# hotchpotch/open_provence

Hardware: AMD Instinct MI355X
Metric: query-context pairs/sec @ seq_len 512, xsmall-v1 (higher is better)
Workload: dtype fp16 single pass (11 significant bits per operand), fp32 accumulate

## Files before the change

### open_provence_amd/csrc/op_api.hip

```cpp
#include "../../include/open_provence_hip.h"

#include <hip/hip_runtime.h>

#include <algorithm>
#include <cmath>
#include <cstdarg>
#include <cstdio>
#include <cstdlib>
#include <cstring>
#include <string>
#include <vector>

#define OPK_PACK_KERNELS 1
#include "op_internal.h"
#include "op_sets.h"
#include "opk_small.hip.h"
#include "opk_padded.hip.h"
#include "opk_tiled.hip.h"

using namespace opk;
using opl::Policy;
using namespace ops;

namespace {
// ... 312 lines not shown
  ChunkPass(op_handle* h_, Launcher& L_, const Workspace& ws_, const int32_t* ids_dev_, const int32_t* cu_dev_, int s0_, int ns_, int rows_,
            int max_len_, int total_tokens_, const AttnPlan& plan_, float* prune_out_, float* rank_out_, float* keep_prob_,
            const HiddenReq* hid_)
      : h(h_), L(L_), ws(ws_), ids_dev(ids_dev_), cu_dev(cu_dev_), s0(s0_), ns(ns_), rows(rows_), max_len(max_len_),
        total_tokens(total_tokens_), plan(plan_), prune_out(prune_out_), rank_out(rank_out_), keep_prob(keep_prob_), hid(hid_) {
    H = h->H;
    I = h->I;
    fp_layout = h->row_path || h->panel_path;
    r_pad = fp_layout ? align_up(rows, ROW_BM) : align_up(rows + 64, 256);
    m_tiles = r_pad / GEMM_BM;
    row_blocks = (unsigned)((r_pad + 3) / 4);
    st = L.stream;
    const KernelSet& ks = *h->ks;
    E = h->eff;
    pi = ks.pi;
    V = opl::kPolicies[pi];
    o_f8 = ks.side == FMT_F8;
    f16 = ks.side == FMT_F16;
    attn16 = o_f8 && ks.attn == FMT_F16;
    auto extra = [](int v, int e, int bit) { return (v & bit) != 0 && (e & bit) == 0; };
    clr_q = !attn16 && extra(V.qk, E.qk, 1);
    clr_k = !attn16 && extra(V.qk, E.qk, 2);
    clr_v = !attn16 && extra(V.pv, E.pv, 2);
    clr_o = extra(V.attn_out, E.attn_out, 1);
    clr_h = extra(V.mlp_out, E.mlp_out, 1);
    clr_ln_attn = extra(V.wqkv, E.wqkv, 1);
    clr_ln_mlp = extra(V.wi, E.wi, 1);
    zero_p_lo = !attn16 && extra(V.pv, E.pv, 1);
    split = (E.wqkv | E.qk | E.pv | E.attn_out | E.wi | E.mlp_out) != 0;
    wi8 = !o_f8 && ks.wi == FMT_F8 && ks.mlp != FMT_F8;
    wlo8 = ks.wlo;
    for (int li = 0; li < h->N; ++li) mlp8[li] = mlp_by_layer(ks) && (li >= 64 || ((h->mlp_layers >> li) & 1ull) != 0);
    range_flagged = h->panel_path && (o_f8 || ks.mlp == FMT_F8);
    fmt_base = f16 ? PF_PK16 : PF_PK;
    fmt_f8 = h->row_path ? PF_ROW_F8A : PF_PANEL16;
    fmt_side = o_f8 ? fmt_f8 : fmt_base;
    fmt_wi = (o_f8 || wi8) ? fmt_f8 : fmt_base;
    embed_in_qkv0 = h->row_path && !h->capture && !(h->cfg.flags & OP_FLAG_NO_HEAD_FUSION);
    plane_bytes = (size_t)r_pad * H * sizeof(u16);
    q_tiles = (max_len + ATT_BQ - 1) / ATT_BQ;
    small_blocks = (r_pad / ROW_BM) <= h->n_cus && !(h->cfg.flags & OP_FLAG_NO_SMALL_BLOCKS);
    row_grid = (unsigned)(r_pad / (small_blocks ? 64 : ROW_BM));
    layer_fused = h->row_path && h->set >= 0 && opl::has_row_layer_fused(pi) && !(h->cfg.flags & OP_FLAG_NO_LAYER_FUSION);
    head_in_last_layer = layer_fused && h->cfg.pooling != OP_POOL_MEAN && !h->capture && !(h->cfg.flags & OP_FLAG_NO_HEAD_FUSION);
    pair_layers = layer_fused && H == 256 && I % 64 == 0 && !split && !h->capture &&
                  !(h->cfg.flags & (OP_FLAG_NO_LAYER_PAIRS | OP_FLAG_LAYER_8X16 | OP_FLAG_LAYER_M32)) &&
                  weight(0, W_ATTN_OUT, f16 ? PF_PAIR16 : PF_PAIR) != nullptr;
  }

  u16* weight(int li, Weight w, PackFmt f) const { return h->layers[li].pack[w][f]; }

  int prologue() {
    OP_TRY(L.begin(PK_ROWMAP));
    hipLaunchKernelGGL(seq_offsets_kernel, dim3(1), dim3(1024), 0, st, cu_dev, s0, ns, ROW_ALIGN, ROW_ALIGN, ws.roff);
    if (fp_layout) {
      hipLaunchKernelGGL(seq_offsets_kernel, dim3(1), dim3(1024), 0, st, cu_dev, s0, ns, plan.waves_g * 32, 1, ws.qboff);
      hipLaunchKernelGGL(seq_offsets_kernel, dim3(1), dim3(1024), 0, st, cu_dev, s0, ns, 128, 1, ws.qboff_l);
    }
    hipLaunchKernelGGL(row_map_kernel, dim3((unsigned)((r_pad + 255) / 256)), dim3(256), 0, st, cu_dev, s0, ns, ws.roff,
                       r_pad, ws.row_seq, ws.row_pos, ws.row_tok);
    OP_TRY(L.end());

    if (range_flagged) OP_HIP(h, hipMemsetAsync(ws.range_flag, 0, sizeof(int), st));
    if (fp_layout && o_f8) {
      const size_t n16 = (size_t)((r_pad - rows) / 16);
      if (n16) OP_HIP(h, hipMemsetAsync(ws.o_hi + (size_t)(rows / 16) * (H / 32) * 512, 0, n16 * (H / 32) * 512 * sizeof(u16), st));
      if (n16) OP_HIP(h, hipMemsetAsync(ws.o_lo + (size_t)(rows / 16) * h->nh * 512, 0, n16 * h->nh * 512 * sizeof(u16), st));
    } else if (fp_layout) {
      const size_t tail_off = (size_t)(rows / 16) * (H / 32) * 2 * 512;
      const size_t tail_bytes = (size_t)((r_pad - rows) / 16) * (H / 32) * 2 * 512 * sizeof(u16);
      if (tail_bytes) OP_HIP(h, hipMemsetAsync(ws.o_hi + tail_off, 0, tail_bytes, st));
    } else {
      const size_t tail_off = (size_t)rows * H;
      const size_t tail_bytes = (size_t)(r_pad - rows) * H * sizeof(u16);
      if (tail_bytes) OP_HIP(h, hipMemsetAsync(ws.o_hi + tail_off, 0, tail_bytes, st));
      if (tail_bytes && split) OP_HIP(h, hipMemsetAsync(ws.o_lo + tail_off, 0, tail_bytes, st));
    }

    if (!embed_in_qkv0) {
      OP_TRY(L.begin(PK_EMBED_LN));
      if (split)
        hipLaunchKernelGGL((embed_ln_kernel<true>), dim3(row_blocks), dim3(256), 0, st, ids_dev, ws.row_tok, h->emb,
                           h->emb_norm, h->cfg.norm_eps, H, r_pad, h->V, ws.x, ws.ln_hi, ws.ln_lo);
      else
        hipLaunchKernelGGL((embed_ln_kernel<false>), dim3(row_blocks), dim3(256), 0, st, ids_dev, ws.row_tok, h->emb,
                           h->emb_norm, h->cfg.norm_eps, H, r_pad, h->V, ws.x, ws.ln_hi, ws.ln_lo);
      OP_TRY(L.end());
    }
    return OP_OK;
  }

  int capture(int index) {
    if (!h->capture) return OP_OK;
    OP_TRY(L.begin(PK_CAPTURE));
    hipLaunchKernelGGL(capture_rows_kernel, dim3(row_blocks), dim3(256), 0, st, ws.x, ws.row_tok, H, r_pad,
                       h->capture + (size_t)index * total_tokens * H);
    return L.end();
  }

  void* hidden_entry(int index) const {
    if (!hid || hid->slot[index] < 0) return nullptr;
    return hid->out + (size_t)hid->slot[index] * hid->entry_bytes;
  }
  int hidden(int index, const float* ln = nullptr) {
    void* dst = hidden_entry(index);
    if (!dst) return OP_OK;
    OP_TRY(L.begin(PK_CAPTURE));
    hipLaunchKernelGGL(hidden_rows_kernel, dim3(row_blocks), dim3(256), 0, st, ws.x, ln, h->cfg.norm_eps, H, r_pad,
                       ws.row_tok, ws.row_seq, ws.row_pos, s0, hid->pad, hid->bf16, dst);
    return L.end();
  }

  int attention(bool is_global) {
// ... 1614 lines not shown
```

### open_provence_amd/csrc/opk_small.hip.h

```cpp
#pragma once

#include "opk_common.hip.h"

namespace opk {

__global__ __launch_bounds__(1024) void seq_offsets_kernel(const int32_t* __restrict__ cu, int s0, int ns, int unit,
                                                           int scale, int32_t* __restrict__ roff) {
  __shared__ int sh[1024];
  __shared__ int carry;
  const int tid = threadIdx.x;
  if (tid == 0) carry = 0;
  __syncthreads();
  for (int base = 0; base < ns; base += 1024) {
    const int i = base + tid;
    int v = 0;
    if (i < ns) {
      const int len = cu[s0 + i + 1] - cu[s0 + i];
      v = (len + unit - 1) / unit * scale;
    }
    sh[tid] = v;
    __syncthreads();
    for (int off = 1; off < 1024; off <<= 1) {
      const int t = tid >= off ? sh[tid - off] : 0;
      __syncthreads();
      sh[tid] += t;
      __syncthreads();
    }
    const int incl = sh[tid];
    const int c = carry;
    if (i < ns) roff[i] = c + incl - v;
    __syncthreads();
    if (tid == 1023) carry = c + incl;
    __syncthreads();
  }
  if (tid == 0) roff[ns] = carry;
}

__global__ void row_map_kernel(const int32_t* __restrict__ cu, int s0, int ns, const int32_t* __restrict__ roff,
                               int r_pad, int32_t* __restrict__ row_seq, int32_t* __restrict__ row_pos,
                               int32_t* __restrict__ row_tok) {
  const int r = blockIdx.x * blockDim.x + threadIdx.x;
  if (r >= r_pad) return;
  const int total = roff[ns];
  if (r >= total) {
    row_seq[r] = -1;
    row_pos[r] = -1;
    row_tok[r] = -1;
    return;
  }
  int lo = 0, hi = ns - 1;
  while (lo < hi) {
    const int mid = (lo + hi + 1) >> 1;
    if (roff[mid] <= r) lo = mid; else hi = mid - 1;
  }
  const int pos = r - roff[lo];
  const int start = cu[s0 + lo];
  const int len = cu[s0 + lo + 1] - start;
  row_seq[r] = lo;
  if (pos < len) {
    row_pos[r] = pos;
    row_tok[r] = start + pos;
  } else {
    row_pos[r] = -1;
    row_tok[r] = -1;
  }
}

constexpr int LN_MAX_CHUNKS = 4;

struct RowVec {
  float4 v[LN_MAX_CHUNKS];
};

__device__ __forceinline__ void row_load(const float* __restrict__ src, int H, int lane, RowVec& rv) {
  const int nchunk = H >> 2;
#pragma unroll
  for (int k = 0; k < LN_MAX_CHUNKS; ++k) {
    const int c = lane + 64 * k;
    rv.v[k] = (c < nchunk) ? reinterpret_cast<const float4*>(src)[c] : make_float4(0.f, 0.f, 0.f, 0.f);
  }
}

__device__ __forceinline__ void row_layer_norm(RowVec& rv, const float* __restrict__ w, int H, int lane, float eps) {
  const int nchunk = H >> 2;
  float s = 0.f;
#pragma unroll
  for (int k = 0; k < LN_MAX_CHUNKS; ++k) s += (rv.v[k].x + rv.v[k].y) + (rv.v[k].z + rv.v[k].w);
  const float mean = wave_sum(s) / (float)H;
  float q = 0.f;
#pragma unroll
  for (int k = 0; k < LN_MAX_CHUNKS; ++k) {
    const int c = lane + 64 * k;
    if (c < nchunk) {
      const float a = rv.v[k].x - mean, b = rv.v[k].y - mean, cc = rv.v[k].z - mean, d = rv.v[k].w - mean;
      q += (a * a + b * b) + (cc * cc + d * d);
    }
  }
  const float var = wave_sum(q) / (float)H;
  const float rstd = 1.0f / sqrtf(var + eps);
#pragma unroll
  for (int k = 0; k < LN_MAX_CHUNKS; ++k) {
    const int c = lane + 64 * k;
    if (c < nchunk) {
      const float4 ww = reinterpret_cast<const float4*>(w)[c];
      rv.v[k].x = (rv.v[k].x - mean) * rstd * ww.x;
      rv.v[k].y = (rv.v[k].y - mean) * rstd * ww.y;
      rv.v[k].z = (rv.v[k].z - mean) * rstd * ww.z;
      rv.v[k].w = (rv.v[k].w - mean) * rstd * ww.w;
    }
  }
}
// ... 99 lines not shown
                                                             const int32_t* __restrict__ row_tok,
                                                             const int32_t* __restrict__ row_seq,
                                                             const int32_t* __restrict__ row_pos,
                                                             const float* __restrict__ pw, const float* __restrict__ pb,
                                                             float* __restrict__ prune_out, float* __restrict__ keep_prob,
                                                             int pre_norm, int keep_all_rows, float* __restrict__ cls,
                                                             float* __restrict__ capture, const int* __restrict__ range_flag) {
  const int lane = threadIdx.x & 63;
  const int row = blockIdx.x * 4 + (threadIdx.x >> 6);
  if (row >= r_pad) return;
  const int tok = row_tok[row];
  if (tok < 0) return;
  RowVec rv;
  row_load(x + (size_t)row * H, H, lane, rv);
  const int nchunk = H >> 2;
  float d0 = 0.f, d1 = 0.f;
  auto head_dot = [&]() {
#pragma unroll
    for (int k = 0; k < LN_MAX_CHUNKS; ++k) {
      const int c = lane + 64 * k;
      if (c < nchunk) {
        const float4 w0 = reinterpret_cast<const float4*>(pw)[c];
        const float4 w1 = reinterpret_cast<const float4*>(pw + H)[c];
        d0 += (rv.v[k].x * w0.x + rv.v[k].y * w0.y) + (rv.v[k].z * w0.z + rv.v[k].w * w0.w);
        d1 += (rv.v[k].x * w1.x + rv.v[k].y * w1.y) + (rv.v[k].z * w1.z + rv.v[k].w * w1.w);
      }
    }
  };
  if (pre_norm) head_dot();
  row_layer_norm(rv, lnw, H, lane, eps);
  if (!pre_norm) head_dot();
  d0 = wave_sum(d0);
  d1 = wave_sum(d1);
  if (lane == 0) {
    const float poison = (range_flag != nullptr && *range_flag != 0) ? __builtin_nanf("") : 0.f;
    const float l0 = d0 + pb[0] + poison, l1 = d1 + pb[1] + poison;
    prune_out[(size_t)tok * 2 + 0] = l0;
    prune_out[(size_t)tok * 2 + 1] = l1;
    if (keep_prob) keep_prob[tok] = 1.0f / (1.0f + expf(l0 - l1));
  }
  if (keep_all_rows) row_store_f32(rv, x + (size_t)row * H, H, lane);
  if (row_pos[row] == 0) row_store_f32(rv, cls + (size_t)row_seq[row] * H, H, lane);
  if (capture) row_store_f32(rv, capture + (size_t)tok * H, H, lane);
}

__device__ __forceinline__ float block_sum_256(float v, float* red) {
  v = wave_sum(v);
  const int wave = threadIdx.x >> 6, lane = threadIdx.x & 63;
  __syncthreads();
  if (lane == 0) red[wave] = v;
  __syncthreads();
  return (red[0] + red[1]) + (red[2] + red[3]);
}

__global__ __launch_bounds__(256) void rank_head_kernel(const float* __restrict__ cls, const float* __restrict__ y,
                                                        const int32_t* __restrict__ cu, int s0,
                                                        const int32_t* __restrict__ roff, int mean_pool, int H, int nl,
                                                        const float* __restrict__ dense_t,
                                                        const float* __restrict__ head_norm, float eps,
                                                        const float* __restrict__ cls_w, const float* __restrict__ cls_b,
                                                        float* __restrict__ rank_out, const int* __restrict__ range_flag) {
  const bool poisoned = range_flag != nullptr && *range_flag != 0;
  __shared__ float pooled[1024];
  __shared__ float z[1024];
  __shared__ float red[4];
  const int s = blockIdx.x;
  const int tid = threadIdx.x;
  const int len = cu[s0 + s + 1] - cu[s0 + s];
  if (len <= 0) {
    if (tid < nl) rank_out[(size_t)(s0 + s) * nl + tid] = 0.f;
    return;
  }
  for (int k = tid; k < H; k += 256) {
    float v;
    if (mean_pool) {
      const float* base = y + (size_t)roff[s] * H + k;
      float acc = 0.f;
      for (int p = 0; p < len; ++p) acc += base[(size_t)p * H];
      v = acc / (float)len;
    } else {
      v = cls[(size_t)s * H + k];
    }
    pooled[k] = v;
  }
  __syncthreads();
  float lsum = 0.f;
  for (int n = tid; n < H; n += 256) {
    float acc = 0.f;
    for (int k = 0; k < H; ++k) acc = fmaf(pooled[k], dense_t[(size_t)k * H + n], acc);
    const float gl = gelu_erf(acc);
    z[n] = gl;
    lsum += gl;
  }
  const float mean = block_sum_256(lsum, red) / (float)H;
  float lq = 0.f;
  for (int n = tid; n < H; n += 256) {
    const float d = z[n] - mean;
    lq += d * d;
  }
  const float var = block_sum_256(lq, red) / (float)H;
  const float rstd = 1.0f / sqrtf(var + eps);
  for (int c = 0; c < nl; ++c) {
    float part = 0.f;
    for (int n = tid; n < H; n += 256) part += (z[n] - mean) * rstd * head_norm[n] * cls_w[(size_t)c * H + n];
    const float tot = block_sum_256(part, red);
    if (tid == 0) rank_out[(size_t)(s0 + s) * nl + c] = poisoned ? __builtin_nanf("") : tot + cls_b[c];
  }
}

__global__ void convert_to_f32_kernel(const void* __restrict__ src, int dtype, size_t n, float* __restrict__ dst) {
  const size_t i = (size_t)blockIdx.x * blockDim.x + threadIdx.x;
  if (i >= n) return;
  if (dtype == 0) {
    dst[i] = reinterpret_cast<const float*>(src)[i];
  } else if (dtype == 1) {
    dst[i] = bf2f(reinterpret_cast<const u16*>(src)[i]);
  } else {
    dst[i] = __half2float(reinterpret_cast<const __half*>(src)[i]);
  }
}

__global__ void split_planes_kernel(const float* __restrict__ src, int rows, int cols, int geglu_half,
                                    u16* __restrict__ hi, u16* __restrict__ lo, int zero_lo, int* __restrict__ any_lo) {
  const size_t i = (size_t)blockIdx.x * blockDim.x + threadIdx.x;
  if (i >= (size_t)rows * cols) return;
  const int r = (int)(i / cols), c = (int)(i % cols);
  int sr = r;
  if (geglu_half > 0) {
    const int b = r >> 6, j = r & 63;
    sr = (j < 32) ? (b * 32 + j) : (geglu_half + b * 32 + (j - 32));
  }
  const float v = src[(size_t)sr * cols + c];
  const u16 h = f2bf(v);
  const u16 l = f2bf(v - bf2f(h));
  if ((l & 0x7fffu) != 0) *any_lo = 1;
  hi[i] = h;
  lo[i] = zero_lo ? (u16)0 : l;
}

__global__ void transpose_f32_kernel(const float* __restrict__ src, int rows, int cols, float* __restrict__ dst) {
  const size_t i = (size_t)blockIdx.x * blockDim.x + threadIdx.x;
  if (i >= (size_t)rows * cols) return;
// ... 198 lines not shown
```

### microbench/rowgemm_ablate.hip

```cpp
#include <hip/hip_runtime.h>

#include <cstdio>
#include <cstring>
#include <cstdlib>
#include <vector>

#include "opk_rowgemm.hip.h"
#include "opk_layer32.hip.h"
#include "opk_layer16p.hip.h"

#ifndef ABL_T
#define ABL_T 1
#endif
#ifndef ABL_NAME
#define ABL_NAME "baseline"
#endif

#define CHECK(x)                                                       \
  do {                                                                 \
    hipError_t e_ = (x);                                               \
    if (e_ != hipSuccess) {                                            \
      fprintf(stderr, "%s: %s\n", #x, hipGetErrorString(e_));          \
      exit(1);                                                         \
    }                                                                  \
// ... 306 lines not shown
      total += (double)(s[last] - s[0]);
      real += (double)s[15];
      ++n;
    }
    printf("  shader clock while the blocks ran: %.3f GHz (cycle stamps / 100 MHz counter)\n", total / real * 0.1);
    printf("  cycles per block (wave 0): attn-out %.0f | residual+LN %.0f | MLP %.0f (of which stage wait+barrier %.0f) | residual+LN %.0f | q/k/v %.0f (vmcnt wait %.0f, barrier %.0f) | total %.0f\n",
           seg[0] / n, seg[1] / n, seg[2] / n, wait / n, seg[3] / n, seg[4] / n, wait1 / n, wait2 / n, total / n);
    double x[4] = {0, 0, 0, 0};
    int nx = 0;
    for (int b = 0; b < blocks; ++b) {
      const unsigned long long* s = &t[(size_t)b * 16];
      if (!s[11] || !s[12]) continue;
      x[0] += (double)(s[11] - (ABL_LAYER == 34 ? s[0] : s[1]));
      x[1] += (double)(s[12] - s[3]);
      x[2] += (double)(s[13] - s[3]);
      x[3] += (double)(s[14] - s[3]);
      ++nx;
    }
#ifdef OPK_SEG_TIMING
    {
      double sg[3] = {0, 0, 0};
      for (int b = 0; b < blocks; ++b)
        for (int i = 0; i < 3; ++i) sg[i] += (double)t[(size_t)b * 16 + 11 + i];
      printf("  MLP loop segments per block: chunk 2t %.0f | chunk 2t+1 + GeGLU %.0f | slab + GeGLU %.0f\n", sg[0] / blocks, sg[1] / blocks, sg[2] / blocks);
    }
    nx = 0;
#endif
    if (nx)
      printf("  LayerNorm 1: row fragment 0 done at +%.0f | LayerNorm 2: fragment 0 +%.0f, arithmetic +%.0f, DMA/RoPE wait +%.0f (then the row stores)\n",
             x[0] / nx, x[1] / nx, x[2] / nx, x[3] / nx);
  }
#endif
#if defined(ABL_LAYER) && ABL_LAYER == 34
  {
    const size_t nx = (size_t)R * H, nq = (size_t)R * H * 2;
    std::vector<float> x1(nx), x2(nx);
    std::vector<u16> q1(nq), q2(nq), k1(nq), k2(nq), v1(nq), v2(nq);
    for (int rep = 0; rep < 2; ++rep) {
      CHECK(hipMemcpy(d_x, x.data(), x.size() * 4, hipMemcpyHostToDevice));
      CHECK(hipMemset(d_q, 0, nq * 2));
      CHECK(hipMemset(d_k, 0, nq * 2));
      CHECK(hipMemset(d_v, 0, nq * 2));
      launch();
      CHECK(hipDeviceSynchronize());
      CHECK(hipMemcpy(rep ? x2.data() : x1.data(), d_x, nx * 4, hipMemcpyDeviceToHost));
      CHECK(hipMemcpy(rep ? q2.data() : q1.data(), d_q, nq * 2, hipMemcpyDeviceToHost));
      CHECK(hipMemcpy(rep ? k2.data() : k1.data(), d_k, nq * 2, hipMemcpyDeviceToHost));
      CHECK(hipMemcpy(rep ? v2.data() : v1.data(), d_v, nq * 2, hipMemcpyDeviceToHost));
    }
    size_t dx = 0, dq = 0, dk = 0, dv = 0, fx = ~(size_t)0, fq = ~(size_t)0;
    for (size_t i = 0; i < nx; ++i) if (memcmp(&x1[i], &x2[i], 4)) { if (!dx) fx = i; ++dx; }
    for (size_t i = 0; i < nq; ++i) { if (q1[i] != q2[i]) { if (!dq) fq = i; ++dq; } dk += k1[i] != k2[i]; dv += v1[i] != v2[i]; }
    printf("  determinism: x differs in %zu of %zu (first %zu), q %zu (first %zu), k %zu, v %zu\n", dx, nx, fx, dq, fq, dk, dv);
    if (dq) {
      size_t h_pw[4] = {0}, h_mf[2] = {0}, h_hf[2] = {0}, h_g[4] = {0}, h_ks[8] = {0}, h_r[4] = {0}, h_n[16] = {0}, h_blk[8] = {0};
      for (size_t i = 0; i < nq; ++i) if (q1[i] != q2[i]) {
        const size_t piece = i / 512, within = i % 512, rb = piece / 16, ks = (piece / 2) % 8, ln = within / 8, e = within % 8;
        h_pw[(rb / 2) % 4]++; h_mf[rb % 2]++; h_hf[(ln / 16) >> 1]++; h_g[2 * ((ln / 16) & 1) + (e >> 2)]++; h_ks[ks]++; h_r[e & 3]++; h_n[ln % 16]++; h_blk[(rb / 8) % 8]++;
      }
      printf("  q diffs by pw:"); for (auto v_ : h_pw) printf(" %zu", v_);
      printf(" | mf:"); for (auto v_ : h_mf) printf(" %zu", v_);
      printf(" | hf:"); for (auto v_ : h_hf) printf(" %zu", v_);
      printf(" | g:"); for (auto v_ : h_g) printf(" %zu", v_);
      printf(" | k-step:"); for (auto v_ : h_ks) printf(" %zu", v_);
      printf(" | r:"); for (auto v_ : h_r) printf(" %zu", v_);
      printf(" | n16:"); for (auto v_ : h_n) printf(" %zu", v_);
      printf(" | block%%8:"); for (auto v_ : h_blk) printf(" %zu", v_);
      printf("\n");
      int shown = 0;
      for (size_t i = 0; i < nq && shown < 12; ++i) if (q1[i] != q2[i]) { printf("    q[%zu] %04x vs %04x\n", i, q1[i], q2[i]); ++shown; }
    }
    if (dv) {
      size_t h_e[8] = {0}, h_kg[4] = {0}, h_n4[4] = {0}, h_d[16] = {0}, h_tok[32] = {0}, h_head[4] = {0};
      for (size_t i = 0; i < nq; ++i) if (v1[i] != v2[i]) {
        const size_t piece = i / 512, within = i % 512, ln = within / 8, e = within % 8;
        h_e[e]++; h_kg[ln / 16]++; h_d[ln % 16]++; h_n4[piece % 4]++; h_tok[(e < 4 ? 0 : 16) + 4 * (ln / 16) + (e & 3)]++;
        h_head[(piece / 8) / (R / 32) % 4]++;
      }
      printf("  v diffs by e:"); for (auto v_ : h_e) printf(" %zu", v_);
      printf(" | kg:"); for (auto v_ : h_kg) printf(" %zu", v_);
      printf(" | n4:"); for (auto v_ : h_n4) printf(" %zu", v_);
      printf(" | head:"); for (auto v_ : h_head) printf(" %zu", v_);
      printf(" | d':"); for (auto v_ : h_d) printf(" %zu", v_);
      printf("\n  v diffs by token of the 32-row tile:"); for (auto v_ : h_tok) printf(" %zu", v_);
      printf("\n");
    }
    if (dx) {
      size_t by_tile[8] = {0}, by_i4[4] = {0}, by_lane_g[4] = {0}, by_rowtile[4] = {0};
      for (size_t i = 0; i < nx; ++i) if (memcmp(&x1[i], &x2[i], 4)) {
        const size_t piece = i / 256, within = i % 256;
        by_i4[piece % 4]++; by_tile[(piece / 4) % 8]++; by_rowtile[(piece / 32) % 4]++; by_lane_g[(within / 4) / 16]++;
      }
      printf("  x diffs by feature tile:"); for (int i = 0; i < 8; ++i) printf(" %zu", by_tile[i]);
      printf(" | by piece (2mf+fh):"); for (int i = 0; i < 4; ++i) printf(" %zu", by_i4[i]);
      printf(" | by lane group g:"); for (int i = 0; i < 4; ++i) printf(" %zu", by_lane_g[i]);
      printf(" | by row tile pw:"); for (int i = 0; i < 4; ++i) printf(" %zu", by_rowtile[i]);
      printf("\n");
    }
  }
#endif
  CHECK(hipGetLastError());
  printf("%-22s terms=%d  avg %.1f us  best %.1f us\n", ABL_NAME, ABL_T, sum / reps * 1e3f, best * 1e3f);
  return 0;
}
```

### open_provence_amd/csrc/opk_layer16p_body.inc

```
  static_assert(NT == 8, "written for hidden = 256");
  static_assert(!HOUT || QKV, "the hidden-state store rides on the q / k / v^T loop's x stores");
  constexpr int H = NT * 32;
  constexpr int KP = NT;
  constexpr int CHUNK = KP * 2 * 512;
  constexpr int SLAB = NT * 2 * 512;
  constexpr int STAGE = 2 * CHUNK + SLAB;
  constexpr int STAGE_B = STAGE * 2;
  constexpr int EXTRA = 16 * 512;
  constexpr int XCH_B = STAGE_B;
  constexpr int HX_B = 2 * STAGE_B;
  constexpr int STAGE_PIECES = STAGE / 512;
  constexpr int O_PIECE0 = 80;
  constexpr int SW_ELEMS = (O_PIECE0 + 64) * 512;
  static_assert(SW_ELEMS >= 2 * STAGE + EXTRA && O_PIECE0 * 512 >= STAGE + 32 * 512, "the o pieces lie behind phase 1's stages");
  __shared__ __attribute__((aligned(16))) u16 sW[SW_ELEMS];
  __shared__ __attribute__((aligned(16))) float sLn[2 * H];
  __shared__ __attribute__((aligned(16))) float sStat[8 * 2 * 16 * 2];

  const int tid = threadIdx.x;
  const int lane = tid & 63;
  const int wave = __builtin_amdgcn_readfirstlane(tid >> 6);
  const int pw = wave & 3, hf = wave >> 2;
  const int n16 = lane & 15, g = lane >> 4;
  const int m0 = blockIdx.x * 128 + pw * 32;
// ... 165 lines not shown
      mean_a[mf] = sum * (1.0f / 128.0f);
      const f32x2 ma2 = f32x2{mean_a[mf], mean_a[mf]};
      f32x2 q4s[4];
#pragma unroll
      for (int i = 0; i < 4; ++i)
#pragma unroll
        for (int q = 0; q < 4; ++q) {
          const f32x2 c = pk_sub(v[i][q], ma2);
          q4s[q] = i == 0 ? pk_mul(c, c) : pk_fma(c, c, q4s[q]);
        }
      const f32x2 qt2 = pk_add(pk_add(q4s[0], q4s[1]), pk_add(q4s[2], q4s[3]));
      float m2 = qt2.x + qt2.y;
      m2 += __shfl_xor(m2, 16, 64);
      m2 += __shfl_xor(m2, 32, 64);
      m2_a[mf] = m2;
      lds_write_f2(stat_addr + (uint32_t)(((wave * 2 + mf) * 16 + n16) * 8), f32x2{mean_a[mf], m2});
    }
    asm volatile("s_waitcnt lgkmcnt(0)" ::: "memory");
    block_barrier();
#ifdef OPK_TIMING
    if (which == 1) opk_x[1] = __builtin_readcyclecounter();
#endif
    const float* lw = &sLn[which * H + 128 * hf + 8 * g];
#pragma unroll
    for (int mf = 0; mf < 2; ++mf) {
      const f32x2 other = lds_read_f2(stat_addr + (uint32_t)((((wave ^ 4) * 2 + mf) * 16 + n16) * 8));
      const float mean = 0.5f * (mean_a[mf] + other.x);
      const float dm = mean_a[mf] - other.x;
      const float m2 = (m2_a[mf] + other.y) + dm * dm * 64.0f;
      const float rstd = 1.0f / sqrtf(m2 * (1.0f / (float)H) + p.eps);
      const f32x2 mn2 = f32x2{mean, mean}, r2 = f32x2{rstd, rstd};
#pragma unroll
      for (int i = 0; i < 4; ++i) {
        const f32x4 w0 = *reinterpret_cast<const f32x4*>(lw + 32 * i);
        const f32x4 w1 = *reinterpret_cast<const f32x4*>(lw + 32 * i + 4);
        const f32x4 t0 = acc1[i][0][mf], t1 = acc1[i][1][mf];
        const f32x2 y0 = pk_mul(pk_mul(pk_sub(f32x2{t0[0], t0[1]}, mn2), r2), f32x2{w0[0], w0[1]});
        const f32x2 y1 = pk_mul(pk_mul(pk_sub(f32x2{t0[2], t0[3]}, mn2), r2), f32x2{w0[2], w0[3]});
        const f32x2 y2 = pk_mul(pk_mul(pk_sub(f32x2{t1[0], t1[1]}, mn2), r2), f32x2{w1[0], w1[1]});
        const f32x2 y3 = pk_mul(pk_mul(pk_sub(f32x2{t1[2], t1[3]}, mn2), r2), f32x2{w1[2], w1[3]});
        a[mf][i] = as_frag(make_uint4(pack2x<H16>(y0.x, y0.y), pack2x<H16>(y1.x, y1.y), pack2x<H16>(y2.x, y2.y), pack2x<H16>(y3.x, y3.y)));
        lds_write_frag(lds0 + (uint32_t)XCH_B + (uint32_t)((wave * 8 + 4 * mf + i) * 1024), a[mf][i]);
      }
    }
    asm volatile("s_waitcnt lgkmcnt(0)" ::: "memory");
    block_barrier();
    const uint32_t oth = lds0 + (uint32_t)XCH_B + (uint32_t)(((wave ^ 4) * 8) * 1024);
    static_for<8>([&](auto f_tag) {
      constexpr int f = decltype(f_tag)::value;
      a[f >> 2][4 + (f & 3)] = lds_read_frag<f * 1024>(oth);
    });
    asm volatile("s_waitcnt lgkmcnt(0)" : "+v"(a[0][4]), "+v"(a[0][5]), "+v"(a[0][6]), "+v"(a[0][7]), "+v"(a[1][4]), "+v"(a[1][5]), "+v"(a[1][6]), "+v"(a[1][7]));
  };
  auto store_rows = [&]() {
#pragma unroll
    for (int i = 0; i < 4; ++i)
#pragma unroll
      for (int mf = 0; mf < 2; ++mf)
#pragma unroll
        for (int fh = 0; fh < 2; ++fh) {
          const f32x4 t = acc1[i][fh][mf];
          store_stream16(XOUT_T ? xtile + i * 1024 + (2 * mf + fh) * 256 : xrow + (size_t)(16 * mf) * H + 32 * i + 4 * fh, make_float4(t[0], t[1], t[2], t[3]));
        }
  };
  const std::true_type yes_{};
  const std::false_type no_{};

  layer_ln(yes_, 0);
  block_barrier();
  const uint32_t hx_pair = lds0 + (uint32_t)HX_B + (uint32_t)((pw * 2) * 1024);
  const uint32_t hx_own = hx_pair + (uint32_t)hf * 8u;
  {
    lds_write_u2(hx_own, 0u, 0u);
    lds_write_u2(hx_own + 1024u, 0u, 0u);
    lds_write_u2(hx_own + 8192u, 0u, 0u);
    lds_write_u2(hx_own + 8192u + 1024u, 0u, 0u);
  }

  f32x4 na[2][2][2];
#pragma unroll
  for (int q = 0; q < 8; ++q) na[q >> 2][(q >> 1) & 1][q & 1] = zero4;
  float gx[8], gq[8];
#pragma unroll
  for (int i = 0; i < 8; ++i) gx[i] = gq[i] = 0.f;
  const uint32_t b_lo = lds0 + (uint32_t)hf * (16384u + 8192u);
  const uint32_t b_hi = lds0 + (uint32_t)hf * (16384u - 8192u);
  const uint32_t b_wo = lds0 + 32768u + (uint32_t)hf * 8192u;
  struct MlpOff {
    static constexpr int at(int s, int j) { return j == 1 ? s * 1024 : (2 * s + (j >> 1)) * 1024; }
    static constexpr int base(int s, int j) { return j == 1 ? 2 : (s < 4 ? 0 : 1); }
  };
  struct WoOff {
    static constexpr int at(int s, int j) { return (2 * s + j) * 1024; }
    static constexpr int base(int, int) { return 0; }
  };
  auto geglu_stage = [&](auto stg_tag, const f32x4 (&src)[2][2], uint32_t dst_addr) {
    constexpr int stg = decltype(stg_tag)::value;
    static_for<8>([&](auto i_tag) {
      constexpr int i = decltype(i_tag)::value, mf = i >> 2, r = i & 3;
      if constexpr (stg == 0) {
        gx[i] = src[0][mf][r];
        gq[i] = gelu_erf_poly(0.f, fabsf(gx[i]), 0);
      } else if constexpr (stg < 5) gq[i] = gelu_erf_poly(gq[i], fabsf(gx[i]), stg);
      else if constexpr (stg == 5) gq[i] = __builtin_amdgcn_exp2f(gq[i]);
      else if constexpr (stg == 6) gq[i] = gelu_erf_finish(gq[i], gx[i]);
      else gq[i] = gq[i] * src[1][mf][r];
    });
    if constexpr (stg == 7) {
      lds_write_u2(dst_addr, pack2x<H16>(gq[0], gq[1]), pack2x<H16>(gq[2], gq[3]));
      lds_write_u2(dst_addr + 1024u, pack2x<H16>(gq[4], gq[5]), pack2x<H16>(gq[6], gq[7]));
    }
  };
  auto interleave6 = [&]() {
#pragma unroll
    for (int i = 0; i < 6; ++i) {
      __builtin_amdgcn_sched_group_barrier(0x008, 1, 0);
      __builtin_amdgcn_sched_group_barrier(0x002, 2, 0);
    }
  };
  auto end_of_stage = [&]() {
#ifdef OPK_TIMING
// ... 30 lines not shown
  asm volatile("s_waitcnt vmcnt(0) lgkmcnt(0)" ::: "memory");
  block_barrier();
  L16P_STAMP(2);
  {
    int t = 0;
    do {
      macro(t, std::integral_constant<int, 0>{});
      macro(t + 1, std::integral_constant<int, 1>{});
      t += 2;
    } while (t < n_it);
  }
  {
    bf16x8 hb[2];
    hb[0] = lds_read_frag<0>(hx_pair);
    hb[1] = lds_read_frag<1024>(hx_pair);
    {
      const uint32_t addr[1] = {b_wo};
      frag_stream_m<4, 2, 1, WoOff, 1>(addr, [&](auto step_tag, bf16x8(&w)[2]) {
        constexpr int s = decltype(step_tag)::value;
        if constexpr (s == 0) asm volatile("" : "+v"(hb[0]), "+v"(hb[1]));
        if constexpr (s < 2) stage_piece(std::integral_constant<int, 4 + s>{}, n_it + 1, 1);
#pragma unroll
        for (int fh = 0; fh < 2; ++fh)
#pragma unroll
          for (int mf = 0; mf < 2; ++mf) acc1[s][fh][mf] = mfma16x<H16>(w[fh], hb[mf], acc1[s][fh][mf]);
        geglu_stage(std::integral_constant<int, 2 * s>{}, na[1], hx_own + 8192u);
        geglu_stage(std::integral_constant<int, 2 * s + 1>{}, na[1], hx_own + 8192u);
      });
    }
    end_of_stage();
    hb[0] = lds_read_frag<0>(hx_pair + 8192u);
    hb[1] = lds_read_frag<1024>(hx_pair + 8192u);
    {
      const uint32_t addr[1] = {b_wo + (uint32_t)STAGE_B};
      frag_stream_m<4, 2, 1, WoOff, 1>(addr, [&](auto step_tag, bf16x8(&w)[2]) {
        constexpr int s = decltype(step_tag)::value;
        if constexpr (s == 0) asm volatile("" : "+v"(hb[0]), "+v"(hb[1]));
#pragma unroll
        for (int fh = 0; fh < 2; ++fh)
#pragma unroll
          for (int mf = 0; mf < 2; ++mf) acc1[s][fh][mf] = mfma16x<H16>(w[fh], hb[mf], acc1[s][fh][mf]);
      });
    }
  }
  block_barrier();
  L16P_STAMP(3);

  if constexpr (!QKV) {
    store_rows();
    L16P_STAMP(4);
  } else {
    constexpr int N_IT = 3 * NT / 2;
    constexpr int N_SW = 2 * NT / 2;
    auto stage_pair = [&](int it, int stage) {
#pragma unroll
      for (int u = 0; u < 4; ++u) {
        const int piece = wave + 8 * u;
        dma_weight(rs_qkv, (uint32_t)(((2 * it) * CHUNK + piece * 512) * 2), stage * STAGE_PIECES + piece);
      }
    };
    stage_pair(0, 0);
    f32x4 rc[2], rs[2];
#pragma unroll
    for (int mf = 0; mf < 2; ++mf) {
      int pos = p.row_pos[m0 + 16 * mf + n16];
      pos = pos < 0 ? 0 : (pos >= p.max_pos ? p.max_pos - 1 : pos);
      rc[mf] = *reinterpret_cast<const f32x4*>(p.rope_cos + (size_t)pos * ROPE_HALF + 16 * hf + 4 * g);
      rs[mf] = *reinterpret_cast<const f32x4*>(p.rope_sin + (size_t)pos * ROPE_HALF + 16 * hf + 4 * g);
    }
    layer_ln(no_, 1);
#ifdef OPK_TIMING
    opk_x[2] = __builtin_readcyclecounter();
#endif
    asm volatile("s_waitcnt vmcnt(0)" ::: "memory");
#ifdef OPK_TIMING
    opk_x[3] = __builtin_readcyclecounter();
#endif
    block_barrier();
    L16P_STAMP(4);

    struct QkvOff {
      static constexpr int at(int s, int j) { return (2 * s + j) * 1024; }
      static constexpr int base(int s, int) { return s < 4 ? 0 : 1; }
    };
    f32x4 qa[2][2][2];
    uint2 st_v[4];
    uint4 st_w[2];
    u16* st_p[2] = {nullptr, nullptr};
    float e_lo[4], e_hi[4];
    auto epilogue_slice = [&](int it, auto sw_tag, auto s_tag, const f32x4 (&c)[2][2]) {
      constexpr bool SW = decltype(sw_tag)::value;
      constexpr int s = decltype(s_tag)::value, mf = s >> 2, r = s & 3;
      if constexpr (SW) {
        const bool is_q = it < N_SW / 2;
        const float qscale = is_q ? 0.125f * 1.44269504088896340736f : 1.0f;
        const float cc = rc[mf][r], ss = rs[mf][r];
        e_lo[r] = rope_lo(c[0][mf][r], c[1][mf][r], cc, ss) * qscale;
        e_hi[r] = rope_hi(c[0][mf][r], c[1][mf][r], cc, ss) * qscale;
        if constexpr (r == 3) {
          st_v[2 * mf] = make_uint2(pack2x<H16>(e_lo[0], e_lo[1]), pack2x<H16>(e_lo[2], e_lo[3]));
          st_v[2 * mf + 1] = make_uint2(pack2x<H16>(e_hi[0], e_hi[1]), pack2x<H16>(e_hi[2], e_hi[3]));
          const int head = is_q ? it : it - N_SW / 2;
          u16* out = is_q ? p.q_fp : p.k_fp;
          st_p[mf] = out + (((rb0 + mf) * NT + 2 * head) * 2) * 512 + (16 * (2 * hf + (g >> 1)) + n16) * 8 + 4 * (g & 1);
        }
      } else {
        if constexpr (s == 7) {
#pragma unroll
          for (int fh = 0; fh < 2; ++fh)
            st_w[fh] = make_uint4(pack2x<H16>(c[fh][0][0], c[fh][0][1]), pack2x<H16>(c[fh][0][2], c[fh][0][3]),
                                  pack2x<H16>(c[fh][1][0], c[fh][1][1]), pack2x<H16>(c[fh][1][2], c[fh][1][3]));
          const size_t tb = (size_t)(m0 >> 5);
          st_p[0] = p.vt_fp + ((((size_t)(it - N_SW) * (size_t)(p.r_pad >> 5) + tb) * 2) * 4 + 2 * hf) * 512 + lane * 8;
        }
      }
    };
    auto epilogue_store = [&](auto sw_tag) {
      constexpr bool SW = decltype(sw_tag)::value;
      if constexpr (SW) {
#pragma unroll
        for (int mf = 0; mf < 2; ++mf) {
          store_stream8(st_p[mf], st_v[2 * mf]);
          store_stream8(st_p[mf] + 1024, st_v[2 * mf + 1]);
        }
      } else {
        store_stream16(st_p[0], st_w[0]);
        store_stream16(st_p[0] + 512, st_w[1]);
      }
    };
    auto interleave4 = [&]() {
#pragma unroll
      for (int i = 0; i < 4; ++i) {
        __builtin_amdgcn_sched_group_barrier(0x008, 1, 0);
        __builtin_amdgcn_sched_group_barrier(0x002, 2, 0);
      }
    };
    auto iteration = [&](auto it_tag, auto first_tag, auto sw_tag, auto swp_tag) {
      constexpr int it = decltype(it_tag)::value, cur = it & 1;
      constexpr bool FIRST = decltype(first_tag)::value, SW = decltype(sw_tag)::value, SWP = decltype(swp_tag)::value;
      constexpr bool XS = it < 8;
      stage_pair(it + 1 < N_IT ? it + 1 : it, cur ^ 1);
      __builtin_amdgcn_sched_barrier(0);
      const uint32_t addr[2] = {b_lo + (uint32_t)(cur * STAGE_B), b_hi + (uint32_t)(cur * STAGE_B)};
      frag_stream_m<8, 2, 2, QkvOff, 2>(addr, [&](auto step_tag, bf16x8(&w)[2]) {
        constexpr int s = decltype(step_tag)::value;
#pragma unroll
        for (int fh = 0; fh < 2; ++fh)
#pragma unroll
          for (int mf = 0; mf < 2; ++mf)
            qa[cur][fh][mf] = SW ? mfma16x<H16>(w[fh], a[mf][s], s == 0 ? zero4 : qa[cur][fh][mf]) : mfma16x<H16>(a[mf][s], w[fh], s == 0 ? zero4 : qa[cur][fh][mf]);
        if constexpr (!FIRST) {
          epilogue_slice(it - 1, swp_tag, step_tag, qa[cur ^ 1]);
          interleave4();
        }
      });
      if constexpr (!FIRST) epilogue_store(swp_tag);
      if constexpr (XS) {
#pragma unroll
        for (int fh = 0; fh < 2; ++fh) {
          const f32x4 t = acc1[it >> 1][fh][it & 1];
          store_stream16(XOUT_T ? xtile + (it >> 1) * 1024 + (2 * (it & 1) + fh) * 256 : xrow + (size_t)(16 * (it & 1)) * H + 32 * (it >> 1) + 4 * fh,
                       make_float4(t[0], t[1], t[2], t[3]));
        }
        if constexpr (HOUT) {
          const int hr = hid_row[it & 1];
          if (hr >= 0) {
#pragma unroll
            for (int fh = 0; fh < 2; ++fh) {
              const f32x4 t = acc1[it >> 1][fh][it & 1];
              const size_t e = (size_t)hr * H + 128 * hf + 8 * g + 32 * (it >> 1) + 4 * fh;
              if (p.hid_bf16)
                store_stream8(reinterpret_cast<u16*>(p.hid_out) + e, make_uint2(pack_bf16x2(t[0], t[1]), pack_bf16x2(t[2], t[3])));
              else
                store_stream16(reinterpret_cast<float*>(p.hid_out) + e, make_float4(t[0], t[1], t[2], t[3]));
            }
          }
        }
      }
      constexpr int N_STORES = (FIRST ? 0 : (SWP ? 4 : 2)) + (XS ? 2 : 0);
      asm volatile("s_waitcnt vmcnt(%0)" ::"n"(N_STORES) : "memory");
      block_barrier();
    };
    iteration(std::integral_constant<int, 0>{}, yes_, yes_, yes_);
    static_for<N_SW - 1>([&](auto j_tag) { iteration(std::integral_constant<int, 1 + decltype(j_tag)::value>{}, no_, yes_, yes_); });
    iteration(std::integral_constant<int, N_SW>{}, no_, no_, yes_);
    static_for<N_IT - N_SW - 1>([&](auto j_tag) { iteration(std::integral_constant<int, N_SW + 1 + decltype(j_tag)::value>{}, no_, no_, no_); });
    static_for<8>([&](auto s_tag) { epilogue_slice(N_IT - 1, no_, s_tag, qa[1]); });
    epilogue_store(no_);
  }
  L16P_STAMP(5);
#ifdef OPK_TIMING
  if (threadIdx.x == 0) {
    for (int i = 0; i < 8; ++i) p.dbg[(size_t)blockIdx.x * 16 + i] = opk_ts[i];
    p.dbg[(size_t)blockIdx.x * 16 + 8] = opk_wait;
    for (int i = 0; i < 4; ++i) p.dbg[(size_t)blockIdx.x * 16 + 11 + i] = opk_x[i];
    p.dbg[(size_t)blockIdx.x * 16 + 15] = wall_clock64() - opk_rt0;
  }
#endif
#undef L16P_STAMP
```

Baseline: 67730.

## Fuse sequence offset scans and row map into one prologue kernel; prefetch rank head weights

Replaces up to three single-block 1024-thread scan launches plus the row_map launch with one multi-block prologue kernel. It computes all three offset prefix sums with wave shuffles, and each block derives its row-to-sequence groups directly instead of binary searching roff. Separately, the rank-head dense GEMV loop is unrolled by 32 with software-prefetched weight loads to hide global memory latency. The fusion removes launch overhead and serialized dependencies in the prologue. The cost is redundant scan work in every block and higher register use in the rank head.

Result: no change. 67420 (-0.5%).

```diff
diff --git a/open_provence_amd/csrc/op_api.hip b/open_provence_amd/csrc/op_api.hip
--- a/open_provence_amd/csrc/op_api.hip
+++ b/open_provence_amd/csrc/op_api.hip
@@ -388,13 +388,9 @@
 
   int prologue() {
     OP_TRY(L.begin(PK_ROWMAP));
-    hipLaunchKernelGGL(seq_offsets_kernel, dim3(1), dim3(1024), 0, st, cu_dev, s0, ns, ROW_ALIGN, ROW_ALIGN, ws.roff);
-    if (fp_layout) {
-      hipLaunchKernelGGL(seq_offsets_kernel, dim3(1), dim3(1024), 0, st, cu_dev, s0, ns, plan.waves_g * 32, 1, ws.qboff);
-      hipLaunchKernelGGL(seq_offsets_kernel, dim3(1), dim3(1024), 0, st, cu_dev, s0, ns, 128, 1, ws.qboff_l);
-    }
-    hipLaunchKernelGGL(row_map_kernel, dim3((unsigned)((r_pad + 255) / 256)), dim3(256), 0, st, cu_dev, s0, ns, ws.roff,
-                       r_pad, ws.row_seq, ws.row_pos, ws.row_tok);
+    hipLaunchKernelGGL(prologue_kernel, dim3((unsigned)((r_pad + ROWMAP_ROWS - 1) / ROWMAP_ROWS)), dim3(ROWMAP_ROWS), 0, st, cu_dev,
+                       s0, ns, plan.waves_g * 32, r_pad, ws.roff, fp_layout ? ws.qboff : nullptr, fp_layout ? ws.qboff_l : nullptr,
+                       ws.row_seq, ws.row_pos, ws.row_tok);
     OP_TRY(L.end());
 
     if (range_flagged) OP_HIP(h, hipMemsetAsync(ws.range_flag, 0, sizeof(int), st));
diff --git a/open_provence_amd/csrc/opk_small.hip.h b/open_provence_amd/csrc/opk_small.hip.h
--- a/open_provence_amd/csrc/opk_small.hip.h
+++ b/open_provence_amd/csrc/opk_small.hip.h
@@ -4,59 +4,110 @@
 
 namespace opk {
 
-__global__ __launch_bounds__(1024) void seq_offsets_kernel(const int32_t* __restrict__ cu, int s0, int ns, int unit,
-                                                           int scale, int32_t* __restrict__ roff) {
-  __shared__ int sh[1024];
-  __shared__ int carry;
-  const int tid = threadIdx.x;
-  if (tid == 0) carry = 0;
-  __syncthreads();
-  for (int base = 0; base < ns; base += 1024) {
+constexpr int ROWMAP_ROWS = 256;
+constexpr int ROWMAP_GROUPS = ROWMAP_ROWS / ROW_ALIGN;
+static_assert(ROWMAP_ROWS % ROW_ALIGN == 0, "a block's rows are whole groups");
+
+__device__ __forceinline__ int wave_scan_incl(int v, int lane) {
+#pragma unroll
+  for (int off = 1; off < 64; off <<= 1) {
+    const int t = __shfl_up(v, off);
+    if (lane >= off) v += t;
+  }
+  return v;
+}
+
+__global__ __launch_bounds__(ROWMAP_ROWS) void prologue_kernel(const int32_t* __restrict__ cu, int s0, int ns, int unit_q,
+                                                               int r_pad, int32_t* __restrict__ roff,
+                                                               int32_t* __restrict__ qboff, int32_t* __restrict__ qboff_l,
+                                                               int32_t* __restrict__ row_seq, int32_t* __restrict__ row_pos,
+                                                               int32_t* __restrict__ row_tok) {
+  __shared__ int wave_tot[4][3];
+  __shared__ int group_seq[ROWMAP_GROUPS], group_off[ROWMAP_GROUPS];
+  const int tid = threadIdx.x, lane = tid & 63, wave = tid >> 6;
+  const int r0 = blockIdx.x * ROWMAP_ROWS;
+  const bool writer = blockIdx.x == 0;
+  const bool blocks = qboff != nullptr;
+  if (tid < ROWMAP_GROUPS) group_seq[tid] = -1;
+  int c_r = 0, c_q = 0, c_l = 0;
+  for (int base = 0; base < ns; base += ROWMAP_ROWS) {
     const int i = base + tid;
-    int v = 0;
+    int v_r = 0, v_q = 0, v_l = 0;
     if (i < ns) {
       const int len = cu[s0 + i + 1] - cu[s0 + i];
-      v = (len + unit - 1) / unit * scale;
-    }
-    sh[tid] = v;
+      v_r = (len + ROW_ALIGN - 1) / ROW_ALIGN * ROW_ALIGN;
+      if (blocks) {
+        v_q = (len + unit_q - 1) / unit_q;
+        v_l = (len + 128 - 1) / 128;
+      }
+    }
+    int e_r = wave_scan_incl(v_r, lane), e_q = 0, e_l = 0;
+    if (blocks) {
+      e_q = wave_scan_incl(v_q, lane);
+      e_l = wave_scan_incl(v_l, lane);
+    }
     __syncthreads();
-    for (int off = 1; off < 1024; off <<= 1) {
-      const int t = tid >= off ? sh[tid - off] : 0;
-      __syncthreads();
-      sh[tid] += t;
-      __syncthreads();
-    }
-    const int incl = sh[tid];
-    const int c = carry;
-    if (i < ns) roff[i] = c + incl - v;
+    if (lane == 63) {
+      wave_tot[wave][0] = e_r;
+      wave_tot[wave][1] = e_q;
+      wave_tot[wave][2] = e_l;
+    }
     __syncthreads();
-    if (tid == 1023) carry = c + incl;
-    __syncthreads();
-  }
-  if (tid == 0) roff[ns] = carry;
-}
-
-__global__ void row_map_kernel(const int32_t* __restrict__ cu, int s0, int ns, const int32_t* __restrict__ roff,
-                               int r_pad, int32_t* __restrict__ row_seq, int32_t* __restrict__ row_pos,
-                               int32_t* __restrict__ row_tok) {
-  const int r = blockIdx.x * blockDim.x + threadIdx.x;
+    int t_r = 0, t_q = 0, t_l = 0;
+#pragma unroll
+    for (int w = 0; w < 4; ++w) {
+      if (w == wave) {
+        e_r += c_r + t_r - v_r;
+        e_q += c_q + t_q - v_q;
+        e_l += c_l + t_l - v_l;
+      }
+      t_r += wave_tot[w][0];
+      t_q += wave_tot[w][1];
+      t_l += wave_tot[w][2];
+    }
+    if (i < ns) {
+      if (writer) {
+        roff[i] = e_r;
+        if (blocks) {
+          qboff[i] = e_q;
+          qboff_l[i] = e_l;
+        }
+      }
+      if (v_r > 0) {
+        const int lo = e_r > r0 ? e_r : r0;
+        const int hi = e_r + v_r < r0 + ROWMAP_ROWS ? e_r + v_r : r0 + ROWMAP_ROWS;
+        for (int r = lo; r < hi; r += ROW_ALIGN) {
+          group_seq[(r - r0) / ROW_ALIGN] = i;
+          group_off[(r - r0) / ROW_ALIGN] = e_r;
+        }
+      }
+    }
+    c_r += t_r;
+    c_q += t_q;
+    c_l += t_l;
+    if (!writer && c_r >= r0 + ROWMAP_ROWS) break;
+  }
+  if (writer && tid == 0) {
+    roff[ns] = c_r;
+    if (blocks) {
+      qboff[ns] = c_q;
+      qboff_l[ns] = c_l;
+    }
+  }
+  __syncthreads();
+  const int r = r0 + tid;
   if (r >= r_pad) return;
-  const int total = roff[ns];
-  if (r >= total) {
+  const int seq = group_seq[tid / ROW_ALIGN];
+  if (seq < 0) {
     row_seq[r] = -1;
     row_pos[r] = -1;
     row_tok[r] = -1;
     return;
   }
-  int lo = 0, hi = ns - 1;
-  while (lo < hi) {
-    const int mid = (lo + hi + 1) >> 1;
-    if (roff[mid] <= r) lo = mid; else hi = mid - 1;
-  }
-  const int pos = r - roff[lo];
-  const int start = cu[s0 + lo];
-  const int len = cu[s0 + lo + 1] - start;
-  row_seq[r] = lo;
+  const int pos = r - group_off[tid / ROW_ALIGN];
+  const int start = cu[s0 + seq];
+  const int len = cu[s0 + seq + 1] - start;
+  row_seq[r] = seq;
   if (pos < len) {
     row_pos[r] = pos;
     row_tok[r] = start + pos;
@@ -262,6 +313,8 @@
   __syncthreads();
   return (red[0] + red[1]) + (red[2] + red[3]);
 }
+
+constexpr int RANK_UNROLL = 32;
 
 __global__ __launch_bounds__(256) void rank_head_kernel(const float* __restrict__ cls, const float* __restrict__ y,
                                                         const int32_t* __restrict__ cu, int s0,
@@ -296,8 +349,26 @@
   __syncthreads();
   float lsum = 0.f;
   for (int n = tid; n < H; n += 256) {
+    const float* __restrict__ wn = dense_t + n;
     float acc = 0.f;
-    for (int k = 0; k < H; ++k) acc = fmaf(pooled[k], dense_t[(size_t)k * H + n], acc);
+    int k = 0;
+    if (H >= RANK_UNROLL) {
+      float cur[RANK_UNROLL], nxt[RANK_UNROLL];
+#pragma unroll
+      for (int j = 0; j < RANK_UNROLL; ++j) cur[j] = wn[(size_t)j * H];
+      for (; k + 2 * RANK_UNROLL <= H; k += RANK_UNROLL) {
+#pragma unroll
+        for (int j = 0; j < RANK_UNROLL; ++j) nxt[j] = wn[(size_t)(k + RANK_UNROLL + j) * H];
+#pragma unroll
+        for (int j = 0; j < RANK_UNROLL; ++j) acc = fmaf(pooled[k + j], cur[j], acc);
+#pragma unroll
+        for (int j = 0; j < RANK_UNROLL; ++j) cur[j] = nxt[j];
+      }
+#pragma unroll
+      for (int j = 0; j < RANK_UNROLL; ++j) acc = fmaf(pooled[k + j], cur[j], acc);
+      k += RANK_UNROLL;
+    }
+    for (; k < H; ++k) acc = fmaf(pooled[k], wn[(size_t)k * H], acc);
     const float gl = gelu_erf(acc);
     z[n] = gl;
     lsum += gl;
```

## Stage QKV weights two iterations at a time in a four-slot LDS ring

Applied to the files above, without the earlier changes.

Replaces the double-buffered per-iteration weight staging for the q/k/v^T projection loop with a four-slot LDS ring. Each even iteration prefetches the next two iterations' weights, so the vmcnt wait and block barrier run only every other iteration. It also routes the x output pointer through an opaque global-address-space cast so the stores can be emitted as global rather than flat stores. This halves barrier count and deepens prefetch, at the cost of more LDS use and a longer, more delicate vmcnt accounting that must stay correct.

New measurement: 67450 before, 68100 after (median of 6 runs). Within noise of the previous version (+1.0%).

```diff
diff --git a/microbench/rowgemm_ablate.hip b/microbench/rowgemm_ablate.hip
--- a/microbench/rowgemm_ablate.hip
+++ b/microbench/rowgemm_ablate.hip
@@ -382,6 +382,15 @@
     for (size_t i = 0; i < nx; ++i) if (memcmp(&x1[i], &x2[i], 4)) { if (!dx) fx = i; ++dx; }
     for (size_t i = 0; i < nq; ++i) { if (q1[i] != q2[i]) { if (!dq) fq = i; ++dq; } dk += k1[i] != k2[i]; dv += v1[i] != v2[i]; }
     printf("  determinism: x differs in %zu of %zu (first %zu), q %zu (first %zu), k %zu, v %zu\n", dx, nx, fx, dq, fq, dk, dv);
+    {
+      auto fnv = [](const void* data, size_t bytes) {
+        unsigned long long h = 1469598103934665603ull;
+        const unsigned char* b = static_cast<const unsigned char*>(data);
+        for (size_t i = 0; i < bytes; ++i) h = (h ^ b[i]) * 1099511628211ull;
+        return h;
+      };
+      printf("  output hashes: x %016llx q %016llx k %016llx v %016llx\n", fnv(x1.data(), nx * 4), fnv(q1.data(), nq * 2), fnv(k1.data(), nq * 2), fnv(v1.data(), nq * 2));
+    }
     if (dq) {
       size_t h_pw[4] = {0}, h_mf[2] = {0}, h_hf[2] = {0}, h_g[4] = {0}, h_ks[8] = {0}, h_r[4] = {0}, h_n[16] = {0}, h_blk[8] = {0};
       for (size_t i = 0; i < nq; ++i) if (q1[i] != q2[i]) {
diff --git a/open_provence_amd/csrc/opk_layer16p_body.inc b/open_provence_amd/csrc/opk_layer16p_body.inc
--- a/open_provence_amd/csrc/opk_layer16p_body.inc
+++ b/open_provence_amd/csrc/opk_layer16p_body.inc
@@ -241,6 +241,8 @@
     });
     asm volatile("s_waitcnt lgkmcnt(0)" : "+v"(a[0][4]), "+v"(a[0][5]), "+v"(a[0][6]), "+v"(a[0][7]), "+v"(a[1][4]), "+v"(a[1][5]), "+v"(a[1][6]), "+v"(a[1][7]));
   };
+  float* xrow_st = xrow;
+  float* xtile_st = xtile;
   auto store_rows = [&]() {
 #pragma unroll
     for (int i = 0; i < 4; ++i)
@@ -249,13 +251,20 @@
 #pragma unroll
         for (int fh = 0; fh < 2; ++fh) {
           const f32x4 t = acc1[i][fh][mf];
-          store_stream16(XOUT_T ? xtile + i * 1024 + (2 * mf + fh) * 256 : xrow + (size_t)(16 * mf) * H + 32 * i + 4 * fh, make_float4(t[0], t[1], t[2], t[3]));
+          store_stream16(XOUT_T ? xtile_st + i * 1024 + (2 * mf + fh) * 256 : xrow_st + (size_t)(16 * mf) * H + 32 * i + 4 * fh, make_float4(t[0], t[1], t[2], t[3]));
         }
   };
   const std::true_type yes_{};
   const std::false_type no_{};
 
   layer_ln(yes_, 0);
+  {
+    typedef __attribute__((address_space(1))) float gfloat;
+    gfloat* xg = (gfloat*)(XOUT_T ? xtile : xrow);
+    asm volatile("" : "+v"(xg));
+    if constexpr (XOUT_T) xtile_st = (float*)xg;
+    else xrow_st = (float*)xg;
+  }
   block_barrier();
   const uint32_t hx_pair = lds0 + (uint32_t)HX_B + (uint32_t)((pw * 2) * 1024);
   const uint32_t hx_own = hx_pair + (uint32_t)hf * 8u;
@@ -392,14 +401,22 @@
   } else {
     constexpr int N_IT = 3 * NT / 2;
     constexpr int N_SW = 2 * NT / 2;
-    auto stage_pair = [&](int it, int stage) {
+    struct QkvRing {
+      static constexpr int piece0(int it) { return (it & 3) == 0 ? 0 : (it & 3) == 1 ? 112 : (it & 3) == 2 ? 48 : 80; }
+      static constexpr int stores(int it) { return (it == 0 ? 0 : (it - 1 < N_SW ? 4 : 2)) + (it < 8 ? 2 : 0); }
+    };
+    static_assert(SW_ELEMS >= (QkvRing::piece0(1) + 32) * 512 && QkvRing::piece0(0) + 32 <= XCH_B / 1024 && QkvRing::piece0(1) * 1024 >= XCH_B + 65536,
+                  "q / k / v^T stages 0 and 1 lie clear of the LayerNorm exchange");
+    auto stage_pair = [&](auto it_tag) {
+      constexpr int it = decltype(it_tag)::value;
 #pragma unroll
       for (int u = 0; u < 4; ++u) {
         const int piece = wave + 8 * u;
-        dma_weight(rs_qkv, (uint32_t)(((2 * it) * CHUNK + piece * 512) * 2), stage * STAGE_PIECES + piece);
-      }
-    };
-    stage_pair(0, 0);
+        dma_weight(rs_qkv, (uint32_t)(((2 * it) * CHUNK + piece * 512) * 2), QkvRing::piece0(it) + piece);
+      }
+    };
+    stage_pair(std::integral_constant<int, 0>{});
+    stage_pair(std::integral_constant<int, 1>{});
     f32x4 rc[2], rs[2];
 #pragma unroll
     for (int mf = 0; mf < 2; ++mf) {
@@ -479,9 +496,12 @@
       constexpr int it = decltype(it_tag)::value, cur = it & 1;
       constexpr bool FIRST = decltype(first_tag)::value, SW = decltype(sw_tag)::value, SWP = decltype(swp_tag)::value;
       constexpr bool XS = it < 8;
-      stage_pair(it + 1 < N_IT ? it + 1 : it, cur ^ 1);
+      if constexpr ((it & 1) == 0 && it + 2 < N_IT) {
+        stage_pair(std::integral_constant<int, it + 2>{});
+        stage_pair(std::integral_constant<int, it + 3>{});
+      }
       __builtin_amdgcn_sched_barrier(0);
-      const uint32_t addr[2] = {b_lo + (uint32_t)(cur * STAGE_B), b_hi + (uint32_t)(cur * STAGE_B)};
+      const uint32_t addr[2] = {b_lo + (uint32_t)(QkvRing::piece0(it) * 1024), b_hi + (uint32_t)(QkvRing::piece0(it) * 1024)};
       frag_stream_m<8, 2, 2, QkvOff, 2>(addr, [&](auto step_tag, bf16x8(&w)[2]) {
         constexpr int s = decltype(step_tag)::value;
 #pragma unroll
@@ -499,7 +519,7 @@
 #pragma unroll
         for (int fh = 0; fh < 2; ++fh) {
           const f32x4 t = acc1[it >> 1][fh][it & 1];
-          store_stream16(XOUT_T ? xtile + (it >> 1) * 1024 + (2 * (it & 1) + fh) * 256 : xrow + (size_t)(16 * (it & 1)) * H + 32 * (it >> 1) + 4 * fh,
+          store_stream16(XOUT_T ? xtile_st + (it >> 1) * 1024 + (2 * (it & 1) + fh) * 256 : xrow_st + (size_t)(16 * (it & 1)) * H + 32 * (it >> 1) + 4 * fh,
                        make_float4(t[0], t[1], t[2], t[3]));
         }
         if constexpr (HOUT) {
@@ -517,9 +537,11 @@
           }
         }
       }
-      constexpr int N_STORES = (FIRST ? 0 : (SWP ? 4 : 2)) + (XS ? 2 : 0);
-      asm volatile("s_waitcnt vmcnt(%0)" ::"n"(N_STORES) : "memory");
-      block_barrier();
+      static_assert(QkvRing::stores(it) == (FIRST ? 0 : (SWP ? 4 : 2)) + (XS ? 2 : 0), "the step's stores as counted");
+      if constexpr ((it & 1) == 1 && it + 1 < N_IT) {
+        asm volatile("s_waitcnt vmcnt(%0)" ::"n"(QkvRing::stores(it - 1) + QkvRing::stores(it)) : "memory");
+        block_barrier();
+      }
     };
     iteration(std::integral_constant<int, 0>{}, yes_, yes_, yes_);
     static_for<N_SW - 1>([&](auto j_tag) { iteration(std::integral_constant<int, 1 + decltype(j_tag)::value>{}, no_, yes_, yes_); });
```
